# ParBLiSS/FastANI

Measured on NVIDIA H100. Metric: genome-pairs/sec (many-to-many, k=16, fragLen=3000), higher is better.
Workload: dtype u64

## Files before the change

fastani_b200/api.py:

```python
import ctypes as C
import os
import weakref
import numpy as np

_HERE = os.path.dirname(os.path.abspath(__file__))
_LIB_PATH = os.path.join(_HERE, "lib", "libfastani_b200.so")
_LIB = None

MAPPING_DTYPE = np.dtype([
    ("queryLen", "<i4"), ("refStartPos", "<i4"), ("refEndPos", "<i4"),
    ("queryStartPos", "<i4"), ("queryEndPos", "<i4"), ("refSeqId", "<i4"),
    ("querySeqId", "<i4"), ("nucIdentity", "<f4"), ("nucIdentityUpperBound", "<f4"),
    ("sketchSize", "<i4"), ("conservedSketches", "<i4")])
MINIMIZER_DTYPE = np.dtype([("hash", "<u4"), ("seqId", "<i4"), ("wpos", "<i4")])
CGI_DTYPE = np.dtype([("refGenomeId", "<i4"), ("qryGenomeId", "<i4"), ("countSeq", "<i4"),
                      ("totalQueryFragments", "<i4"), ("identity", "<f4")])
FRAG_DTYPE = np.dtype([("qryGenomeId", "<i4"), ("querySeqId", "<i4"), ("refSeqId", "<i4"), ("refStartPos", "<i4"),
                       ("identity", "<f4")])


class BaniError(RuntimeError):
    def __init__(self, code, msg):
        super().__init__("fastani_b200 error %d: %s" % (code, msg))
        self.code = code
# ... 45 lines not shown
        "bani_ctx_profile_read": (C.c_int, [vp, vp, vp, vp, vp, i32, P(i32)]),
        "bani_ctx_path_counts": (C.c_int, [vp, vp, vp, i32, P(i32)]),
        "bani_host_alloc": (C.c_int, [C.c_size_t, P(vp)]),
        "bani_host_free": (None, [vp]),
        "bani_genome_create": (C.c_int, [vp, i32, vp, vp, P(vp)]),
        "bani_genome_create_batch": (C.c_int, [vp, i32, vp, vp, vp, P(vp)]),
        "bani_pack_contig": (C.c_int, [vp, i64, vp, vp, vp, u64, P(u64)]),
        "bani_genome_create_packed_batch": (C.c_int, [vp, i32, vp, vp, vp, vp, vp, vp, vp, i32, P(vp)]),
        "bani_genome_destroy": (None, [vp]),
        "bani_genome_info": (C.c_int, [vp, P(i32), P(u64), P(u64), P(u64)]),
        "bani_genome_decode": (C.c_int, [vp, vp, i32, vp, i64]),
        "bani_index_build": (C.c_int, [vp, P(vp), i32, P(vp)]),
        "bani_index_destroy": (None, [vp]),
        "bani_index_stats": (C.c_int, [vp, P(u64), P(u64), P(u64), P(u64), P(u64)]),
        "bani_index_minimizers": (C.c_int, [vp, vp, vp, u64]),
        "bani_index_save": (C.c_int, [vp, vp, C.c_char_p]),
        "bani_index_load": (C.c_int, [vp, C.c_char_p, P(vp)]),
        "bani_index_contigs": (C.c_int, [vp, vp, u64, vp, u64]),
        "bani_qsketch_from_index": (C.c_int, [vp, vp, vp, i32, vp, P(vp)]),
        "bani_index_lookup": (C.c_int, [vp, vp, u32, vp, vp, u64, P(u64)]),
        "bani_map_genome": (C.c_int, [vp, vp, vp, P(vp), P(u64), P(u64), P(MapCounters)]),
        "bani_map_cgi": (C.c_int, [vp, vp, P(vp), i32, P(vp), P(u64), vp, P(MapCounters)]),
        "bani_device_count": (C.c_int, [P(i32)]),
        "bani_qsketch_create": (C.c_int, [vp, P(vp), i32, vp, vp, P(vp)]),
        "bani_qsketch_destroy": (None, [vp]),
        "bani_qsketch_info": (C.c_int, [vp, P(i32), P(u64), P(u64), P(u64)]),
        "bani_qsketch_export": (C.c_int, [vp, vp, vp, u64]),
        "bani_qsketch_import": (C.c_int, [vp, vp, u64, P(vp)]),
        "bani_qsketch_merge": (C.c_int, [vp, P(vp), i32, P(vp)]),
        "bani_map_cgi_sketch": (C.c_int, [vp, vp, P(vp), i32, P(vp), P(u64), P(MapCounters)]),
# ... 17 lines not shown
        "bani_qsketch_from_index_file": (C.c_int, [vp, C.c_char_p, vp, i32, vp, P(vp)]),
    }
    for name, (res, args) in sig.items():
        fn = getattr(L, name)
        fn.restype = res
        fn.argtypes = args
    _LIB = L
    return L


EXPORTED_SYMBOLS = [
    "bani_last_error", "bani_version", "bani_params_default", "bani_recommended_window_size", "bani_device_count",
    "bani_stat_min_hits_relaxed", "bani_stat_identity", "bani_ctx_create", "bani_ctx_destroy", "bani_ctx_params",
    "bani_ctx_sync", "bani_ctx_stream", "bani_ctx_launch_count", "bani_ctx_set_flag", "bani_ctx_profile_enable", "bani_ctx_profile_read", "bani_ctx_path_counts", "bani_host_alloc", "bani_host_free", "bani_genome_create",
    "bani_genome_create_batch", "bani_pack_contig", "bani_genome_create_packed_batch", "bani_genome_destroy", "bani_genome_info", "bani_genome_decode", "bani_index_build",
    "bani_index_destroy", "bani_index_stats", "bani_index_minimizers", "bani_index_save", "bani_index_load", "bani_index_contigs",
    "bani_qsketch_from_index", "bani_index_lookup", "bani_map_genome",
    "bani_map_cgi", "bani_free", "bani_synth_genome", "bani_qsketch_create", "bani_qsketch_destroy", "bani_qsketch_info",
    "bani_qsketch_export", "bani_qsketch_import", "bani_qsketch_merge", "bani_map_cgi_sketch", "bani_map_cgi_sketch_frags",
    "bani_index_build_budget", "bani_ctx_mem_stats", "bani_ctx_trim", "bani_ctx_plan_run", "bani_plan_run", "bani_run_working_set", "bani_index_footprint",
    "bani_map_working_set", "bani_index_budget", "bani_plan_chunks", "bani_qsketch_bytes_estimate", "bani_parse_byte_count",
    "bani_index_file_info", "bani_index_load_budget", "bani_qsketch_from_index_file"]


def _check(rc):
    if rc != 0:
        raise BaniError(rc, load_library().bani_last_error().decode())


def _records_from(ptr, n, dtype):
    out = np.empty(int(n), dtype)
# ... 293 lines not shown
        nc = st["n_contigs"]
        sk.metadata = [((names[c] if names else ""), int(cl[c])) for c in range(nc)]
        sk.sequencesByFileInfo = [int(x) for x in sbf[:st["n_genomes"]]]
        return sk

    def stats(self):
        a = [C.c_uint64() for _ in range(5)]
        _check(self.ctx.lib.bani_index_stats(self.h, *[C.byref(x) for x in a]))
        return dict(zip(("n_minimizers", "n_unique", "total_len", "n_contigs", "n_genomes"), [x.value for x in a]))

    def minimizerIndex(self):
        n = self.stats()["n_minimizers"]
        out = np.empty(max(n, 1), MINIMIZER_DTYPE)
        _check(self.ctx.lib.bani_index_minimizers(self.ctx.h, self.h, out.ctypes.data, n))
        return out[:n]

    def lookup(self, hash_value, cap=1 << 16):
        s = np.empty(cap, np.int32); w = np.empty(cap, np.int32); n = C.c_uint64()
        _check(self.ctx.lib.bani_index_lookup(self.ctx.h, self.h, int(hash_value), s.ctypes.data, w.ctypes.data, cap, C.byref(n)))
        m = min(n.value, cap)
        return list(zip(s[:m].tolist(), w[:m].tolist())), n.value

    def sanityCheck(self, maxRatioDiff):
        st = self.stats()
        if st["n_minimizers"] == 0 or st["n_unique"] == 0:
            return True, np.float32(0)
        hashRatio = np.float32(st["total_len"]) / np.float32(st["n_minimizers"])
        uniqHashRatio = np.float32(st["total_len"]) / np.float32(st["n_unique"])
        diff = np.float32(abs(hashRatio - uniqHashRatio))
        return (not diff > np.float32(maxRatioDiff)), diff
# ... 301 lines not shown
```

fastani_b200/csrc/budget.cpp:

```cpp
#include "common.cuh"
#include <algorithm>

namespace bani {

IndexFootprint index_footprint(uint64_t M, uint64_t Ub, uint64_t nC, uint64_t bits, uint64_t stagingCap)
{
  auto R = [](uint64_t b) { return (uint64_t)dev_round_size((size_t)b); };
  Ub = std::min(Ub, M);
  const uint64_t tables = R(4 * (nC + 1)) + R(4 * std::max<uint64_t>(nC, 1)) + R(4 * (nC + 1)) + (nC ? R(8 * nC) : 0);
  const uint64_t bitmap = R(4 * (bits / 32 + 1));
  const uint64_t desc = R(sizeof(SeqDesc) * std::max<uint64_t>(nC, 1));
  const uint64_t rec4 = R(4 * M);
  const uint64_t sketchTemp = R(4 * (nC + 1)) + R(2 * stagingCap + 8 * nC + 16);
  const uint64_t sketchStage = 2 * tables + 2 * bitmap + desc + 3 * R(4 * stagingCap) + sketchTemp + 3 * rec4;
  const uint64_t cubSort = R(8 * M + M / 4 + ((uint64_t)64 << 20));
  const uint64_t cubScan = R(M / 64 + ((uint64_t)1 << 20));
  const int fb = index_filt_bits(Ub);
  const uint64_t lookup = R(4 * Ub) + R(4 * (Ub + 1)) + R(4 * ((1ull << index_dir_bits(Ub)) + 1)) + R(32ull << index_tab_bits(Ub)) +
                          (fb ? R(4ull << (fb - 5)) : 0);
  const uint64_t l2 = R(16 * M) + R(8 * M) + R(8 * M) + R(4 * ((M + 1023) / 1024));
  const uint64_t base = tables + bitmap + 3 * rec4 + 2 * rec4;
  const uint64_t finishStage = base + 4 * rec4 + R(8) + std::max(std::max(cubSort, cubScan), lookup + l2);
  IndexFootprint f;
  f.peak = std::max(sketchStage, finishStage);
  f.resident = base + lookup + l2;
  return f;
}

uint64_t map_working_set(uint64_t deviceBytes, long long maxHitsPerPiece, long long eventBytesPerPiece)
{
  const uint64_t hits = 12ull * (uint64_t)std::max(1ll, maxHitsPerPiece);
  const uint64_t events = eventBytesPerPiece > 0 ? (uint64_t)eventBytesPerPiece : deviceBytes / 4;
  return hits + events + (3ull << 30);
}

uint64_t map_working_set_run(uint64_t deviceBytes, long long maxHitsPerPiece, long long eventBytesPerPiece, uint64_t queryHashes,
                             uint64_t queryFragments, uint64_t nQueries, uint64_t refBases, uint64_t nRefs, int w, int fragLen)
// ... 131 lines not shown
```

fastani_b200/csrc/capi.cu:

```cuda
#include "common.cuh"
#include <algorithm>
#include <cstring>
#include <cstdlib>

struct bani_ctx    { bani::Ctx c; };
struct bani_genome { bani::Genome g; };
struct bani_index  { bani::Index *ix; };
struct bani_qsketch { bani::QSketch *qs; };

namespace bani {
static thread_local std::string g_err;
void set_last_error(const std::string &m) { g_err = m; }
const char *const PATH_NAMES[NPATH] = {
  "l1.class0", "l1.class1", "l1.class2", "l1.class3", "l1.class4", "l1.class5", "l1.class6", "l1.class7", "l1.class8",
  "l1.class9", "l1.class10", "l1.class11", "l1.class12", "l1.device_wide",
  "lookup.walk_saturated", "lookup.walk_full_bucket",
  "l2.events_nt64", "l2.events_nt128", "l2.events_nt256", "l2.dir1024", "l2.dir4096", "l2.staged", "l2.direct",
  "l2.exact_at_bounds", "l2.exact_total",
  "piece.mapped", "piece.split_hits", "piece.split_events", "cgi.passes", "cgi.sparse"};
}

using namespace bani;

#define BANI_TRY try {
// ... 625 lines not shown
  const Index *ix = ixh->ix;
  if (cap < ix->M) fail(BANI_ERR_ARG, "output buffer too small (%llu < %llu)", (unsigned long long)cap, (unsigned long long)ix->M);
  BANI_CUDA(cudaSetDevice(ctx->c.device));
  const size_t M = ix->M;
  if (!M) return BANI_OK;
  std::vector<uint32_t> h(M); std::vector<int32_t> s(M), w(M);
  BANI_CUDA(cudaStreamSynchronize(ctx->c.stream));
  BANI_CUDA(cudaMemcpy(h.data(), ix->hash.p, 4 * M, cudaMemcpyDeviceToHost));
  BANI_CUDA(cudaMemcpy(s.data(), ix->seqId.p, 4 * M, cudaMemcpyDeviceToHost));
  BANI_CUDA(cudaMemcpy(w.data(), ix->wpos.p, 4 * M, cudaMemcpyDeviceToHost));
  for (size_t i = 0; i < M; i++) { out[i].hash = h[i]; out[i].seqId = s[i]; out[i].wpos = w[i]; }
  return BANI_OK;
  BANI_CATCH
}

int bani_index_lookup(bani_ctx *ctx, const bani_index *ixh, uint32_t hash, int32_t *seqId, int32_t *wpos, uint64_t cap, uint64_t *n)
{
  BANI_TRY
  if (!ctx || !ixh || !ixh->ix || !n) fail(BANI_ERR_ARG, "null argument");
  const Index *ix = ixh->ix;
  BANI_CUDA(cudaSetDevice(ctx->c.device));
  BANI_CUDA(cudaStreamSynchronize(ctx->c.stream));
  *n = 0;
  if (!ix->U) return BANI_OK;
  const uint32_t b = hash >> (32 - ix->dirBits);
  uint32_t d[2];
  BANI_CUDA(cudaMemcpy(d, ix->dir.p + b, 8, cudaMemcpyDeviceToHost));
  if (d[1] <= d[0]) return BANI_OK;
  std::vector<uint32_t> keys(d[1] - d[0]);
  BANI_CUDA(cudaMemcpy(keys.data(), ix->ukeys.p + d[0], 4 * keys.size(), cudaMemcpyDeviceToHost));
// ... 210 lines not shown
```

fastani_b200/csrc/common.cuh:

```cuda
#pragma once
#include <cuda_runtime.h>
#include <stdint.h>
#include <string>
#include <vector>
#include <memory>
#include <map>
#include <stdexcept>
#include <cstdio>
#include <cstdarg>
#include <chrono>
#include "../../include/fastani_b200.h"

namespace bani {

struct Error : std::runtime_error {
  int code;
  Error(int c, const std::string &m) : std::runtime_error(m), code(c) {}
};

void set_last_error(const std::string &m);

[[noreturn]] inline void fail(int code, const char *fmt, ...)
{
  char buf[512];
// ... 340 lines not shown
                  int64_t len, uint8_t *hostOut);

size_t cub_sort_pairs_u32_temp(size_t n);
void   cub_sort_pairs_u32(void *temp, size_t tempBytes, const uint32_t *kin, uint32_t *kout,
                          const uint32_t *vin, uint32_t *vout, size_t n, int endBit, cudaStream_t s);
size_t cub_sort_keys_u64_temp(size_t n);
void   cub_sort_keys_u64(void *temp, size_t tempBytes, const uint64_t *kin, uint64_t *kout, size_t n,
                         int beginBit, int endBit, cudaStream_t s);
size_t cub_sort_pairs_u64_u32_temp(size_t n);
void   cub_sort_pairs_u64_u32(void *temp, size_t tempBytes, const uint64_t *kin, uint64_t *kout,
                              const uint32_t *vin, uint32_t *vout, size_t n, int endBit, cudaStream_t s);
size_t cub_scan_u32_temp(size_t n);
void   cub_exclusive_sum_u32(void *temp, size_t tempBytes, const uint32_t *in, uint32_t *out, size_t n, cudaStream_t s);
size_t cub_scan_u64_temp(size_t n);
void   cub_exclusive_sum_u32_to_u64(void *temp, size_t tempBytes, const uint32_t *in, uint64_t *out, size_t n, cudaStream_t s);

}
```

fastani_b200/csrc/cubops.cu:

```cuda
#include <cub/cub.cuh>
#include "common.cuh"

namespace bani {

size_t cub_sort_pairs_u32_temp(size_t n)
{
  size_t b = 0;
  cub::DeviceRadixSort::SortPairs(nullptr, b, (const uint32_t *)nullptr, (uint32_t *)nullptr,
                                  (const uint32_t *)nullptr, (uint32_t *)nullptr, n);
  return b;
}
void cub_sort_pairs_u32(void *temp, size_t tempBytes, const uint32_t *kin, uint32_t *kout,
                        const uint32_t *vin, uint32_t *vout, size_t n, int endBit, cudaStream_t s)
{
  BANI_CUDA(cub::DeviceRadixSort::SortPairs(temp, tempBytes, kin, kout, vin, vout, n, 0, endBit, s));
}
size_t cub_sort_keys_u64_temp(size_t n)
{
  size_t b = 0;
  cub::DeviceRadixSort::SortKeys(nullptr, b, (const uint64_t *)nullptr, (uint64_t *)nullptr, n);
  return b;
}
void cub_sort_keys_u64(void *temp, size_t tempBytes, const uint64_t *kin, uint64_t *kout, size_t n,
                       int beginBit, int endBit, cudaStream_t s)
// ... 24 lines not shown
}
struct U32toU64 { __host__ __device__ uint64_t operator()(uint32_t x) const { return (uint64_t)x; } };
size_t cub_scan_u64_temp(size_t n)
{
  size_t b = 0;
  cub::TransformInputIterator<uint64_t, U32toU64, const uint32_t *> it((const uint32_t *)nullptr, U32toU64());
  cub::DeviceScan::ExclusiveSum(nullptr, b, it, (uint64_t *)nullptr, n);
  return b;
}
void cub_exclusive_sum_u32_to_u64(void *temp, size_t tempBytes, const uint32_t *in, uint64_t *out, size_t n, cudaStream_t s)
{
  cub::TransformInputIterator<uint64_t, U32toU64, const uint32_t *> it(in, U32toU64());
  BANI_CUDA(cub::DeviceScan::ExclusiveSum(temp, tempBytes, it, out, n, s));
}

}
```

fastani_b200/csrc/index.cu:

```cuda
#include "common.cuh"
#include <algorithm>

namespace bani {

static inline unsigned nblk(uint64_t n, int t = 256) { return (unsigned)((n + t - 1) / t); }

__global__ void iota_kernel(uint32_t *v, uint64_t n)
{
  uint64_t i = (uint64_t)blockIdx.x * blockDim.x + threadIdx.x;
  if (i < n) v[i] = (uint32_t)i;
}

__global__ void head_flags_kernel(const uint32_t *sh, uint64_t n, uint32_t *head)
{
  uint64_t i = (uint64_t)blockIdx.x * blockDim.x + threadIdx.x;
  if (i < n) head[i] = (i == 0 || sh[i] != sh[i - 1]) ? 1u : 0u;
}

__global__ void unique_scatter_kernel(const uint32_t *sh, const uint32_t *head, const uint32_t *scan, uint64_t n,
                                      uint32_t *ukeys, uint32_t *uoff, unsigned long long *o_U)
{
  uint64_t i = (uint64_t)blockIdx.x * blockDim.x + threadIdx.x;
  if (i >= n) return;
  if (head[i]) { ukeys[scan[i]] = sh[i]; uoff[scan[i]] = (uint32_t)i; }
  if (i == n - 1) { uint32_t U = scan[i] + head[i]; *o_U = U; }
}

__global__ void links_kernel(const uint32_t *sh, const uint32_t *posIdx, uint64_t n, uint32_t *link)
{
  uint64_t i = (uint64_t)blockIdx.x * blockDim.x + threadIdx.x;
  if (i >= n) return;
  const uint32_t h = sh[i];
  const bool hasPrev = i > 0 && sh[i - 1] == h, hasNext = i + 1 < n && sh[i + 1] == h;
  if (!hasPrev && !hasNext) return;
  const uint32_t r = posIdx[i];
  uint32_t pd = 0xFFFFu, nd = 0xFFFFu;
  if (hasPrev) pd = min(r - posIdx[i - 1], 0xFFFFu);
  if (hasNext) nd = min(posIdx[i + 1] - r, 0xFFFFu);
  if (pd != 0xFFFFu || nd != 0xFFFFu) link[r] = (pd << 16) | nd;
}

__global__ void zip_records_kernel(const uint32_t *hash, const int32_t *wpos, const uint32_t *link, const int32_t *seqId,
                                   const uint32_t *contigRecOff, int cmw, uint64_t n, uint4 *rec, int2 *pos8, uint2 *rec8)
{
  uint64_t i64 = (uint64_t)blockIdx.x * blockDim.x + threadIdx.x;
  if (i64 >= n) return;
  const uint32_t i = (uint32_t)i64;
  const int32_t wx = wpos[i];
  const int seq = seqId[i];
  const uint32_t lo = contigRecOff[seq], hi = contigRecOff[seq + 1];
  uint32_t back = 0, fwd = 0xFFFFu, tie = 0;
  if (cmw >= 2) {
    {
      const int32_t v = wx - cmw + 1;
      uint32_t l = (i - lo > (uint32_t)cmw) ? i - (uint32_t)cmw : lo, h = i;
      while (l < h) { uint32_t m = (l + h) >> 1; if (wpos[m] <= v) l = m + 1; else h = m; }
      back = min(i - l + 1, 0xFFFFu);
    }
    if (i + 1 < hi) {
      const int32_t v = wpos[i + 1] + cmw - 1;
      uint32_t l = i + 1, h = (hi - i - 1 > (uint32_t)cmw + 1) ? i + 1 + (uint32_t)cmw + 1 : hi;
      while (l < h) { uint32_t m = (l + h) >> 1; if (wpos[m] < v) l = m + 1; else h = m; }
      fwd = min(l - i, 0xFFFEu);
      tie = (l < hi && wpos[l] == v) ? 1u : 0u;
    }
  }
  rec[i] = make_uint4(hash[i], (uint32_t)wx | (tie << 31), link[i], back | (fwd << 16));
  pos8[i] = make_int2(wx, seq);
  const uint32_t pd = link[i] >> 16, nd = link[i] & 0xFFFFu;
  const uint32_t f14 = fwd == 0xFFFFu ? 0x3FFFu : min(fwd, 0x3FFEu);
  rec8[i] = make_uint2(hash[i], (back & 0x3FFFu) | (f14 << 14) | (tie << 28) | ((pd > back ? 1u : 0u) << 29) | ((nd >= fwd ? 1u : 0u) << 30));
}

__global__ void block_link_max_kernel(const uint4 *rec, uint64_t n, uint32_t *blkMax)
{
  __shared__ uint32_t s_b, s_f;
  if (threadIdx.x == 0) { s_b = 0; s_f = 0; }
  __syncthreads();
  uint32_t mb = 0, mf = 0;
  for (int j = 0; j < 4; j++) {
    const uint64_t i = (uint64_t)blockIdx.x * 1024 + (uint64_t)j * 256 + threadIdx.x;
    if (i < n) {
      const uint32_t w = rec[i].w, back = w & 0xFFFFu, fwd = w >> 16;
      if (back >= 0x3FFFu || (fwd != 0xFFFFu && fwd >= 0x3FFFu)) { mb = 0xFFFFu; mf = 0xFFFFu; }
      else { mb = max(mb, back); if (fwd != 0xFFFFu) mf = max(mf, fwd); }
    }
  }
  atomicMax(&s_b, mb); atomicMax(&s_f, mf);
  __syncthreads();
  if (threadIdx.x == 0) blkMax[blockIdx.x] = min(s_b, 0xFFFFu) | (min(s_f, 0xFFFFu) << 16);
}

__global__ void dir_fill_kernel(const uint32_t *ukeys, uint32_t U, int dirBits, uint32_t *dir)
{
  uint32_t b = blockIdx.x * blockDim.x + threadIdx.x;
  if (b > (1u << dirBits)) return;
  uint32_t lo = 0, hi = U;
  if (b == (1u << dirBits)) lo = U;
  else { const uint32_t v = b << (32 - dirBits); while (lo < hi) { uint32_t mid = (lo + hi) >> 1; if (ukeys[mid] < v) lo = mid + 1; else hi = mid; } }
  dir[b] = lo;
}

__global__ void table_fill_kernel(const uint32_t *ukeys, const uint32_t *uoff, uint32_t U, uint32_t mask, uint2 *tab,
                                  uint32_t *filt, uint32_t filtMask)
{
  const uint32_t u = blockIdx.x * blockDim.x + threadIdx.x;
  if (u >= U) return;
  const uint32_t h = ukeys[u], o = uoff[u], cnt = uoff[u + 1] - o;
  if (filt) atomicOr(&filt[(h & filtMask) >> 5], 1u << (h & 31u));
  const unsigned long long e = ((unsigned long long)o << 32) | (unsigned long long)((h & 0xFFFFFF00u) | min(cnt, 255u));
  unsigned long long *bp = reinterpret_cast<unsigned long long *>(tab + 4 * (size_t)(h & mask));
#pragma unroll
  for (int sl = 0; sl < 4; sl++) if (atomicCAS(bp + sl, 0ull, e) == 0ull) return;
}

__global__ void fill_u32(uint32_t *p, uint32_t v, uint64_t n)
{
  uint64_t i = (uint64_t)blockIdx.x * blockDim.x + threadIdx.x;
  if (i < n) p[i] = v;
}

static unsigned long long index_contig_tables(Ctx *ctx, Index *ix, const std::vector<int32_t> &contigGenome)
{
  cudaStream_t st = ctx->stream;
  const int fragLen = ix->fragLen;
  const int32_t nC = (int32_t)ix->contigLen.size();
  std::vector<uint32_t> binOff(1, 0);
  std::vector<unsigned long long> bitBase;
// ... 33 lines not shown
  BANI_CUDA(cudaMemsetAsync(ix->dir.p, 0, 4 * ((1u << ix->dirBits) + 1), st));
  ix->ukeys.alloc(1, st); ix->uoff.alloc(2, st); ix->posIdx.alloc(1, st);
  BANI_CUDA(cudaMemsetAsync(ix->uoff.p, 0, 8, st));
  ix->tabBits = 8; ix->tab.alloc((size_t)4 << ix->tabBits, st);
  BANI_CUDA(cudaMemsetAsync(ix->tab.p, 0, ix->tab.bytes(), st));
  ix->hash.alloc(1, st); ix->wpos.alloc(1, st); ix->seqId.alloc(1, st); ix->link.alloc(1, st);
  BANI_CUDA(cudaStreamSynchronize(st));
}

static void index_finish(Ctx *ctx, Index *ix)
{
  cudaStream_t st = ctx->stream;
  const uint64_t M = ix->M;
  ix->link.alloc(M, st);
  ix->posIdx.alloc(M, st);
  DevBuf<uint32_t> sortedHash(M, st), iota(M, st), head(M, st), scan(M, st);
  DevBuf<unsigned long long> d_U(1, st);
  {
    Stage sg(ctx, "index_sort", 24.0 * M);
    iota_kernel<<<nblk(M), 256, 0, st>>>(iota.p, M);
    ctx->launches++;
    size_t tb = cub_sort_pairs_u32_temp(M);
    DevBuf<uint8_t> tmp(tb, st);
    cub_sort_pairs_u32(tmp.p, tb, ix->hash.p, sortedHash.p, iota.p, ix->posIdx.p, M, 32, st);
  }
  Stage sgc(ctx, "index_compact", 16.0 * M);
  head_flags_kernel<<<nblk(M), 256, 0, st>>>(sortedHash.p, M, head.p);
  ctx->launches++;
  {
    size_t tb = cub_scan_u32_temp(M);
    DevBuf<uint8_t> tmp(tb, st);
    cub_exclusive_sum_u32(tmp.p, tb, head.p, scan.p, M, st);
  }
  uint32_t lastScan = 0, lastHead = 0;
  BANI_CUDA(cudaMemcpyAsync(&lastScan, scan.p + (M - 1), 4, cudaMemcpyDeviceToHost, st));
  BANI_CUDA(cudaMemcpyAsync(&lastHead, head.p + (M - 1), 4, cudaMemcpyDeviceToHost, st));
  BANI_CUDA(cudaStreamSynchronize(st));
  const uint64_t U = (uint64_t)lastScan + lastHead;
  ix->U = U;
  ix->ukeys.alloc(U, st); ix->uoff.alloc(U + 1, st);
  unique_scatter_kernel<<<nblk(M), 256, 0, st>>>(sortedHash.p, head.p, scan.p, M, ix->ukeys.p, ix->uoff.p, d_U.p);
  ctx->launches++;
  { uint32_t Mu = (uint32_t)M; BANI_CUDA(cudaMemcpyAsync(ix->uoff.p + U, &Mu, 4, cudaMemcpyHostToDevice, st)); }
  BANI_CUDA(cudaMemsetAsync(ix->link.p, 0xFF, 4 * (size_t)M, st));
  links_kernel<<<nblk(M), 256, 0, st>>>(sortedHash.p, ix->posIdx.p, M, ix->link.p);
  ctx->launches++;
  const int bits = index_dir_bits(U);
  ix->dirBits = bits;
  ix->dir.alloc((1u << bits) + 1, st);
  dir_fill_kernel<<<nblk((1ull << bits) + 1), 256, 0, st>>>(ix->ukeys.p, (uint32_t)U, bits, ix->dir.p);
  ctx->launches++;
  {
    const int tb = index_tab_bits(U);
    ix->tabBits = tb;
    ix->tab.alloc((size_t)4 << tb, st);
    BANI_CUDA(cudaMemsetAsync(ix->tab.p, 0, ix->tab.bytes(), st));
    const int fb = index_filt_bits(U);
    ix->filtBits = fb;
    if (fb) { ix->filt.alloc((size_t)1 << (fb - 5), st); BANI_CUDA(cudaMemsetAsync(ix->filt.p, 0, ix->filt.bytes(), st)); }
    table_fill_kernel<<<nblk(U), 256, 0, st>>>(ix->ukeys.p, ix->uoff.p, (uint32_t)U, (1u << tb) - 1u, ix->tab.p,
                                               ix->filt.p, fb ? (uint32_t)((1ull << fb) - 1ull) : 0u);
    ctx->launches++;
  }
  ix->rec.alloc(M, st);
  ix->cmw = ix->fragLen - (ix->w - 1) - (ix->k - 1);
  ix->pos8.alloc(M, st); ix->rec8.alloc(M, st);
  zip_records_kernel<<<nblk(M), 256, 0, st>>>(ix->hash.p, ix->wpos.p, ix->link.p, ix->seqId.p, ix->contigRecOff.p, ix->cmw, M, ix->rec.p, ix->pos8.p, ix->rec8.p);
  ctx->launches++;
  ix->blkMax.alloc((size_t)((M + 1023) / 1024), st);
  block_link_max_kernel<<<(unsigned)((M + 1023) / 1024), 256, 0, st>>>(ix->rec.p, M, ix->blkMax.p);
  ctx->launches++;
  sgc.stop();
  BANI_CUDA(cudaGetLastError());
  BANI_CUDA(cudaStreamSynchronize(st));
}

struct GenomeSpan { uint64_t nC = 0, pos = 0, bits = 0; };
static GenomeSpan genome_span(const Genome *G, int k)
{
  GenomeSpan s;
  s.nC = (uint64_t)G->nContigs;
  for (int c = 0; c < G->nContigs; c++) {
    if (G->len[c] >= k) s.pos += (uint64_t)(G->len[c] - k + 1);
    s.bits += ((uint64_t)G->len[c] + 31) & ~31ull;
  }
// ... 98 lines not shown
  const int32_t nC = (int32_t)desc.size();
  ctx->mark("index_build: enter + contig loop");
  const unsigned long long totalBits = index_contig_tables(ctx, ix.get(), contigGenome);
  ctx->mark("index_build: contig tables");

  if (nC == 0 || totalPos == 0) { index_make_empty(ctx, ix.get()); return ix.release(); }

  ix->validBits.alloc((size_t)(totalBits / 32) + 1, st);
  BANI_CUDA(cudaMemsetAsync(ix->validBits.p, 0, ix->validBits.bytes(), st));
  DevBuf<SeqDesc> d_desc(nC, st);
  BANI_CUDA(cudaMemcpyAsync(d_desc.p, desc.data(), sizeof(SeqDesc) * (size_t)nC, cudaMemcpyHostToDevice, st));

  uint64_t cap = index_staging_cap(totalPos, w);
  uint64_t M = 0;
  {
    DevBuf<uint32_t> th; DevBuf<int32_t> tw, ts;
    std::vector<std::pair<int32_t, int32_t>> groups;
    std::vector<const Genome *> groupHead;
    {
      int32_t c = 0;
      for (int g = 0; g < nRefs; g++) {
        const Genome *G = refs[g];
        const bool newGroup = groups.empty() || G->blk != groupHead.back()->blk;
        if (newGroup) { groups.push_back({c, c}); groupHead.push_back(G); }
        c += G->nContigs; groups.back().second = c;
      }
    }
    for (int attempt = 0; attempt < 2; attempt++) {
      if (cap > 0xfffffff0ull) fail(BANI_ERR_LIMIT, "more than 2^32 minimizers in one index shard");
      th.alloc(cap, st); tw.alloc(cap, st); ts.alloc(cap, st);
      Stage sg(ctx, "ref_sketch", (double)ix->totalLen / 4.0);
      M = 0;
      for (size_t gi = 0; gi < groups.size(); gi++) {
        const int32_t ca = groups[gi].first, cb = groups[gi].second;
        groupHead[gi]->wait_ready(st);
        M += sketch_sequences(ctx, d_desc.p + ca, cb - ca, ix->contigLen.data() + ca, 0, th.p, tw.p, ts.p, cap, ix->contigRecOff.p + ca,
                              ix->validBits.p, ix->contigBitBase.p + ca, M);
        if (M > 0xfffffff0ull) fail(BANI_ERR_LIMIT, "more than 2^32 minimizers in one index shard");
      }
      sg.bytes((double)ix->totalLen / 4.0 + 12.0 * (double)M);
      ctx->mark("index_build: sketched");
      if (M <= cap) break;
      if (budget) {
        uint32_t r1 = 0;
        BANI_CUDA(cudaMemcpyAsync(&r1, ix->contigRecOff.p + ix->seqsByFile[0], 4, cudaMemcpyDeviceToHost, st));
        BANI_CUDA(cudaStreamSynchronize(st));
        if (r1 <= cap) break;
        if (index_footprint(r1, r1, (uint64_t)nC, totalBits, r1).peak > maxBytes)
          fail(BANI_ERR_LIMIT, "reference genome 0 of this chunk (%llu minimizers) does not fit the index budget of %llu bytes",
               (unsigned long long)r1, (unsigned long long)maxBytes);
        cap = r1;
        continue;
      }
      cap = M;
    }
    d_desc.release();
    if (budget) M = index_cut(ctx, ix.get(), refs, contigGenome, span, std::min(M, cap), cap, maxBytes, nTaken);
    if (M > 0xfffffff0ull) fail(BANI_ERR_LIMIT, "more than 2^32 minimizers in one index shard");
    ix->M = M;
    if (M == 0) { index_make_empty(ctx, ix.get()); return ix.release(); }
    ix->hash.alloc(M, st); ix->wpos.alloc(M, st); ix->seqId.alloc(M, st);
    BANI_CUDA(cudaMemcpyAsync(ix->hash.p, th.p, 4 * M, cudaMemcpyDeviceToDevice, st));
    BANI_CUDA(cudaMemcpyAsync(ix->wpos.p, tw.p, 4 * M, cudaMemcpyDeviceToDevice, st));
    BANI_CUDA(cudaMemcpyAsync(ix->seqId.p, ts.p, 4 * M, cudaMemcpyDeviceToDevice, st));
  }
  index_finish(ctx, ix.get());
  ctx->mark("index_build: finished");
  return ix.release();
}

Index *index_build(Ctx *ctx, Genome *const *refs, int32_t nRefs)
{
  int32_t n = 0;
  return index_build_impl(ctx, refs, nRefs, 0, &n);
}

template <typename F>
static Index *with_peak(Ctx *ctx, uint64_t *peakBytes, F &&make)
{
// ... 7 lines not shown
  dev_mem_peak_set(ctx->device, std::max(peak0, peak));
  *peakBytes = peak > live0 ? peak - live0 : 0;
  return ix;
}

Index *index_build_budget(Ctx *ctx, Genome *const *refs, int32_t nRefs, uint64_t maxBytes, int32_t *nTaken, uint64_t *peakBytes)
{
  if (nRefs < 1) fail(BANI_ERR_ARG, "a budgeted index build needs at least one genome");
  if (maxBytes == 0) fail(BANI_ERR_ARG, "the index budget must be positive");
  return with_peak(ctx, peakBytes, [&] { return index_build_impl(ctx, refs, nRefs, maxBytes, nTaken); });
}


static constexpr uint64_t IX_MAGIC = 0x32584449494e4142ull;
static constexpr uint64_t IX_HEADER_BYTES = 128;

__global__ void seqid_fill_kernel(const uint32_t *contigRecOff, int32_t nC, int32_t *seqId)
{
  const int c = blockIdx.x;
  if (c >= nC) return;
  const uint32_t a = contigRecOff[c], b = contigRecOff[c + 1];
  for (uint32_t i = a + threadIdx.x; i < b; i += blockDim.x) seqId[i] = c;
}

static uint64_t word_sum(const void *p, size_t bytes)
{
  const uint32_t *w = (const uint32_t *)p;
  uint64_t s = 0;
  for (size_t i = 0; i < bytes / 4; i++) s += w[i];
  return s;
}

namespace {
struct File {
  FILE *f = nullptr; std::string path; uint64_t sum = 0;
  File(const char *p, const char *mode) : f(fopen(p, mode)), path(p) { if (!f) fail(BANI_ERR_ARG, "cannot open %s", p); }
  ~File() { if (f) fclose(f); }
  void write(const void *p, size_t n) { if (n && fwrite(p, 1, n, f) != n) fail(BANI_ERR_INTERNAL, "write error on %s", path.c_str()); sum += word_sum(p, n); }
// ... 322 lines not shown
```

fastani_b200/csrc/sketch.cu:

```cuda
#include "common.cuh"

namespace bani {

static constexpr int SK_THREADS = 256;
static constexpr int SK_P = 16;
static constexpr int SK_SLOTS = SK_THREADS * SK_P;
static constexpr int SK_WMAX = 1024;
static constexpr int SK_KMAX = 32;
static constexpr int SK_ASCII = SK_SLOTS + SK_KMAX + 64;
#define KIDX(q) ((q) + ((q) >> 4))
static constexpr int SK_KEYS = SK_SLOTS + SK_SLOTS / 16;

struct SketchArgs {
  const SeqDesc *desc; const uint32_t *tileOff;
  int32_t nSeq; uint32_t nTiles;
  int32_t uniformTiles;
  int k, w, tileLen;
  uint32_t *o_hash; int32_t *o_wpos; int32_t *o_seqId; uint64_t cap;
  uint32_t *o_segStart;
  unsigned long long *tileState;
  unsigned long long *o_total;
  uint32_t *o_validBits; const unsigned long long *bitBase;
  unsigned long long recBase;
};
// ... 99 lines not shown
  }
}

__device__ __forceinline__ uint64_t min64(uint64_t a, uint64_t b) { return a < b ? a : b; }

__device__ __forceinline__ void expand8(uint32_t x, uint32_t &b0, uint32_t &b1)
{
  x = (x | (x << 8)) & 0x00FF00FFu;
  x = (x | (x << 4)) & 0x0F0F0F0Fu;
  x = (x | (x << 2)) & 0x33333333u;
  b0 = __byte_perm(0x54474341u, 0u, x & 0xFFFFu);
  b1 = __byte_perm(0x54474341u, 0u, x >> 16);
}

template <int KT, int G>
__global__ void __launch_bounds__(SK_THREADS)
sketch_kernel(const SketchArgs a)
{
  __shared__ __align__(16) uint8_t  s_ascii[SK_ASCII];
  __shared__ __align__(16) uint64_t s_key[SK_KEYS];
  __shared__ uint16_t s_vmask[SK_THREADS];
  __shared__ uint32_t s_wsum[SK_THREADS / 32];
  __shared__ unsigned long long s_base;

  const int tid = threadIdx.x, lane = tid & 31, wid = tid >> 5;
  const uint32_t tile = blockIdx.x;
  const int k = KT > 0 ? KT : a.k, w = a.w;

  int seq, t0;
  if (a.uniformTiles > 0) { seq = (int)(tile / (uint32_t)a.uniformTiles); t0 = (int)(tile % (uint32_t)a.uniformTiles) * a.tileLen; }
  else {
// ... 242 lines not shown
```

include/fastani_b200.h:

```cpp
#ifndef FASTANI_B200_H
#define FASTANI_B200_H

#include <stdint.h>
#include <stddef.h>

#ifdef __cplusplus
extern "C" {
#endif

#define BANI_API __attribute__((visibility("default")))

typedef enum {
  BANI_OK = 0,
  BANI_ERR_ARG = -1,
  BANI_ERR_CUDA = -2,
  BANI_ERR_NOMEM = -3,
  BANI_ERR_LIMIT = -4,
  BANI_ERR_INTERNAL = -5
} bani_status;

typedef struct {
  int32_t  kmer_size;
  int32_t  window_size;
  int32_t  frag_len;
// ... 99 lines not shown
                               uint64_t budget, int32_t *chunk_end, int32_t *n_chunks);
BANI_API int  bani_qsketch_bytes_estimate(uint64_t len, int32_t w, int32_t frag_len, uint64_t *bytes);
BANI_API int  bani_plan_run(uint64_t free_bytes, uint64_t device_bytes, int64_t max_hits_per_piece, int64_t event_bytes_per_piece,
                            uint64_t index_budget, uint64_t query_budget, int32_t k, int32_t w, int32_t frag_len,
                            const uint64_t *ref_len, const int32_t *ref_contigs, int32_t n_refs, const uint64_t *query_len,
                            const uint64_t *query_sketch_bytes, int32_t n_queries, int32_t *chunk_end, int32_t *n_chunks,
                            int32_t *block_end, int32_t *n_blocks, uint64_t *index_budget_used);
BANI_API int  bani_ctx_plan_run(bani_ctx *ctx, uint64_t index_budget, uint64_t query_budget, const uint64_t *ref_len, const int32_t *ref_contigs, int32_t n_refs,
                                const uint64_t *query_len, const uint64_t *query_sketch_bytes, int32_t n_queries,
                                int32_t *chunk_end, int32_t *n_chunks, int32_t *block_end, int32_t *n_blocks,
                                uint64_t *index_budget_used);
BANI_API int  bani_parse_byte_count(const char *s, uint64_t *out);
BANI_API int  bani_index_stats(const bani_index *ix, uint64_t *n_minimizers, uint64_t *n_unique,
                               uint64_t *total_len, uint64_t *n_contigs, uint64_t *n_genomes);
BANI_API int  bani_index_minimizers(bani_ctx *ctx, const bani_index *ix, bani_minimizer *out, uint64_t cap);
BANI_API int  bani_index_lookup(bani_ctx *ctx, const bani_index *ix, uint32_t hash,
                                int32_t *seqId, int32_t *wpos, uint64_t cap, uint64_t *n);

BANI_API int  bani_index_save(bani_ctx *ctx, const bani_index *ix, const char *path);
BANI_API int  bani_index_load(bani_ctx *ctx, const char *path, bani_index **out);
BANI_API int  bani_index_contigs(const bani_index *ix, int32_t *contig_len, uint64_t cap_contigs, int32_t *seqs_by_file, uint64_t cap_genomes);

BANI_API int  bani_index_file_info(const char *path, int32_t *version, int32_t *k, int32_t *w, int32_t *frag_len, int32_t *n_genomes,
                                   uint64_t *n_contigs, uint64_t *n_minimizers, int32_t *genome_contigs, uint64_t *genome_len,
                                   uint64_t *genome_records, uint64_t *genome_bits, uint64_t cap_genomes, int32_t *contig_len,
                                   uint64_t cap_contigs);
BANI_API int  bani_index_load_budget(bani_ctx *ctx, const char *path, int32_t first_genome, uint64_t max_bytes, bani_index **out,
                                     int32_t *n_taken, uint64_t *peak_bytes);

BANI_API int  bani_map_genome(bani_ctx *ctx, const bani_index *ix, const bani_genome *query,
// ... 36 lines not shown
```

Baseline: 2.112 million.

## Streamline index build: CUB unique, fused zip/blkMax, seqId fill, sketch bounds

Replaces the head-flag, scan and scatter sequence in index compaction with a CUB run-count followed by UniqueByKey. Fuses the block link-max reduction into the record zip kernel, which now handles 1024 elements per block with warp reductions. Drops the per-minimizer seqId staging buffer from sketching and rebuilds seqId from contig offsets. It also adds min-blocks 4 to the sketch kernel's launch bounds, which may cause register spills, and adds an index-array export API. These mostly cut index-build launches, memory and traffic, which is a small share of many-to-many mapping throughput.

New measurement: 2.150 million, median of 6. 1.02x the previous value.

```diff
diff --git a/fastani_b200/api.py b/fastani_b200/api.py
--- a/fastani_b200/api.py
+++ b/fastani_b200/api.py
@@ -83,6 +83,7 @@
         "bani_index_destroy": (None, [vp]),
         "bani_index_stats": (C.c_int, [vp, P(u64), P(u64), P(u64), P(u64), P(u64)]),
         "bani_index_minimizers": (C.c_int, [vp, vp, vp, u64]),
+        "bani_index_array": (C.c_int, [vp, vp, C.c_char_p, vp, u64, P(u64)]),
         "bani_index_save": (C.c_int, [vp, vp, C.c_char_p]),
         "bani_index_load": (C.c_int, [vp, C.c_char_p, P(vp)]),
         "bani_index_contigs": (C.c_int, [vp, vp, u64, vp, u64]),
@@ -130,7 +131,7 @@
     "bani_stat_min_hits_relaxed", "bani_stat_identity", "bani_ctx_create", "bani_ctx_destroy", "bani_ctx_params",
     "bani_ctx_sync", "bani_ctx_stream", "bani_ctx_launch_count", "bani_ctx_set_flag", "bani_ctx_profile_enable", "bani_ctx_profile_read", "bani_ctx_path_counts", "bani_host_alloc", "bani_host_free", "bani_genome_create",
     "bani_genome_create_batch", "bani_pack_contig", "bani_genome_create_packed_batch", "bani_genome_destroy", "bani_genome_info", "bani_genome_decode", "bani_index_build",
-    "bani_index_destroy", "bani_index_stats", "bani_index_minimizers", "bani_index_save", "bani_index_load", "bani_index_contigs",
+    "bani_index_destroy", "bani_index_stats", "bani_index_minimizers", "bani_index_array", "bani_index_save", "bani_index_load", "bani_index_contigs",
     "bani_qsketch_from_index", "bani_index_lookup", "bani_map_genome",
     "bani_map_cgi", "bani_free", "bani_synth_genome", "bani_qsketch_create", "bani_qsketch_destroy", "bani_qsketch_info",
     "bani_qsketch_export", "bani_qsketch_import", "bani_qsketch_merge", "bani_map_cgi_sketch", "bani_map_cgi_sketch_frags",
@@ -454,6 +455,13 @@
         out = np.empty(max(n, 1), MINIMIZER_DTYPE)
         _check(self.ctx.lib.bani_index_minimizers(self.ctx.h, self.h, out.ctypes.data, n))
         return out[:n]
+
+    def array(self, name, dtype):
+        n = C.c_uint64()
+        _check(self.ctx.lib.bani_index_array(self.ctx.h, self.h, name.encode(), None, 0, C.byref(n)))
+        out = np.empty(max(n.value, 1), np.uint8)
+        _check(self.ctx.lib.bani_index_array(self.ctx.h, self.h, name.encode(), out.ctypes.data, n.value, C.byref(n)))
+        return out[:n.value].view(dtype)
 
     def lookup(self, hash_value, cap=1 << 16):
         s = np.empty(cap, np.int32); w = np.empty(cap, np.int32); n = C.c_uint64()
diff --git a/fastani_b200/csrc/budget.cpp b/fastani_b200/csrc/budget.cpp
--- a/fastani_b200/csrc/budget.cpp
+++ b/fastani_b200/csrc/budget.cpp
@@ -12,15 +12,16 @@
   const uint64_t desc = R(sizeof(SeqDesc) * std::max<uint64_t>(nC, 1));
   const uint64_t rec4 = R(4 * M);
   const uint64_t sketchTemp = R(4 * (nC + 1)) + R(2 * stagingCap + 8 * nC + 16);
-  const uint64_t sketchStage = 2 * tables + 2 * bitmap + desc + 3 * R(4 * stagingCap) + sketchTemp + 3 * rec4;
+  const uint64_t sketchStage = 2 * tables + 2 * bitmap + desc + 2 * R(4 * stagingCap) + sketchTemp + 3 * rec4;
   const uint64_t cubSort = R(8 * M + M / 4 + ((uint64_t)64 << 20));
-  const uint64_t cubScan = R(M / 64 + ((uint64_t)1 << 20));
+  const uint64_t cubUnique = R(M / 64 + ((uint64_t)1 << 20));
   const int fb = index_filt_bits(Ub);
   const uint64_t lookup = R(4 * Ub) + R(4 * (Ub + 1)) + R(4 * ((1ull << index_dir_bits(Ub)) + 1)) + R(32ull << index_tab_bits(Ub)) +
                           (fb ? R(4ull << (fb - 5)) : 0);
   const uint64_t l2 = R(16 * M) + R(8 * M) + R(8 * M) + R(4 * ((M + 1023) / 1024));
   const uint64_t base = tables + bitmap + 3 * rec4 + 2 * rec4;
-  const uint64_t finishStage = base + 4 * rec4 + R(8) + std::max(std::max(cubSort, cubScan), lookup + l2);
+  const uint64_t compact = cubUnique + R(4) + R(4 * Ub) + R(4 * (Ub + 1));
+  const uint64_t finishStage = base + rec4 + std::max(std::max(rec4 + cubSort, compact), lookup + l2);
   IndexFootprint f;
   f.peak = std::max(sketchStage, finishStage);
   f.resident = base + lookup + l2;
diff --git a/fastani_b200/csrc/capi.cu b/fastani_b200/csrc/capi.cu
--- a/fastani_b200/csrc/capi.cu
+++ b/fastani_b200/csrc/capi.cu
@@ -663,6 +663,29 @@
   BANI_CATCH
 }
 
+int bani_index_array(bani_ctx *ctx, const bani_index *ixh, const char *name, void *out, uint64_t cap_bytes, uint64_t *n_bytes)
+{
+  BANI_TRY
+  if (!ctx || !ixh || !ixh->ix || !name || !n_bytes) fail(BANI_ERR_ARG, "null argument");
+  const Index *ix = ixh->ix;
+  const std::string nm(name);
+  const void *p = nullptr; size_t b = 0; bool found = false;
+  auto pick = [&](const char *n, const auto &buf) { if (nm == n) { p = buf.p; b = buf.bytes(); found = true; } };
+  pick("hash", ix->hash); pick("wpos", ix->wpos); pick("seqId", ix->seqId); pick("link", ix->link); pick("posIdx", ix->posIdx);
+  pick("ukeys", ix->ukeys); pick("uoff", ix->uoff); pick("dir", ix->dir); pick("rec", ix->rec); pick("pos8", ix->pos8);
+  pick("rec8", ix->rec8); pick("blkMax", ix->blkMax); pick("contigRecOff", ix->contigRecOff); pick("tab", ix->tab);
+  pick("filt", ix->filt); pick("validBits", ix->validBits);
+  if (!found) fail(BANI_ERR_ARG, "unknown index array '%s'", name);
+  *n_bytes = b;
+  if (!out) return BANI_OK;
+  if (cap_bytes < b) fail(BANI_ERR_ARG, "output buffer too small (%llu < %llu)", (unsigned long long)cap_bytes, (unsigned long long)b);
+  BANI_CUDA(cudaSetDevice(ctx->c.device));
+  BANI_CUDA(cudaStreamSynchronize(ctx->c.stream));
+  if (b) BANI_CUDA(cudaMemcpy(out, p, b, cudaMemcpyDeviceToHost));
+  return BANI_OK;
+  BANI_CATCH
+}
+
 int bani_index_lookup(bani_ctx *ctx, const bani_index *ixh, uint32_t hash, int32_t *seqId, int32_t *wpos, uint64_t cap, uint64_t *n)
 {
   BANI_TRY
diff --git a/fastani_b200/csrc/common.cuh b/fastani_b200/csrc/common.cuh
--- a/fastani_b200/csrc/common.cuh
+++ b/fastani_b200/csrc/common.cuh
@@ -378,5 +378,10 @@
 void   cub_exclusive_sum_u32(void *temp, size_t tempBytes, const uint32_t *in, uint32_t *out, size_t n, cudaStream_t s);
 size_t cub_scan_u64_temp(size_t n);
 void   cub_exclusive_sum_u32_to_u64(void *temp, size_t tempBytes, const uint32_t *in, uint64_t *out, size_t n, cudaStream_t s);
-
-}
+size_t cub_count_runs_u32_temp(size_t n);
+void   cub_count_runs_u32(void *temp, size_t tempBytes, const uint32_t *keys, uint32_t *o_runs, size_t n, cudaStream_t s);
+size_t cub_unique_u32_temp(size_t n);
+void   cub_unique_u32(void *temp, size_t tempBytes, const uint32_t *keys, uint32_t *o_keys, uint32_t *o_first, uint32_t *o_count,
+                      size_t n, cudaStream_t s);
+
+}
diff --git a/fastani_b200/csrc/cubops.cu b/fastani_b200/csrc/cubops.cu
--- a/fastani_b200/csrc/cubops.cu
+++ b/fastani_b200/csrc/cubops.cu
@@ -62,4 +62,34 @@
   BANI_CUDA(cub::DeviceScan::ExclusiveSum(temp, tempBytes, it, out, n, s));
 }
 
+struct RunHead {
+  const uint32_t *k;
+  __host__ __device__ uint32_t operator()(uint32_t i) const { return (i == 0 || k[i] != k[i - 1]) ? 1u : 0u; }
+};
+size_t cub_count_runs_u32_temp(size_t n)
+{
+  size_t b = 0;
+  cub::TransformInputIterator<uint32_t, RunHead, cub::CountingInputIterator<uint32_t>> it(cub::CountingInputIterator<uint32_t>(0), RunHead{nullptr});
+  cub::DeviceReduce::Sum(nullptr, b, it, (uint32_t *)nullptr, (uint32_t)n);
+  return b;
 }
+void cub_count_runs_u32(void *temp, size_t tempBytes, const uint32_t *keys, uint32_t *o_runs, size_t n, cudaStream_t s)
+{
+  cub::TransformInputIterator<uint32_t, RunHead, cub::CountingInputIterator<uint32_t>> it(cub::CountingInputIterator<uint32_t>(0), RunHead{keys});
+  BANI_CUDA(cub::DeviceReduce::Sum(temp, tempBytes, it, o_runs, (uint32_t)n, s));
+}
+size_t cub_unique_u32_temp(size_t n)
+{
+  size_t b = 0;
+  cub::DeviceSelect::UniqueByKey(nullptr, b, (const uint32_t *)nullptr, cub::CountingInputIterator<uint32_t>(0), (uint32_t *)nullptr,
+                                 (uint32_t *)nullptr, (uint32_t *)nullptr, (uint32_t)n);
+  return b;
+}
+void cub_unique_u32(void *temp, size_t tempBytes, const uint32_t *keys, uint32_t *o_keys, uint32_t *o_first, uint32_t *o_count,
+                    size_t n, cudaStream_t s)
+{
+  BANI_CUDA(cub::DeviceSelect::UniqueByKey(temp, tempBytes, keys, cub::CountingInputIterator<uint32_t>(0), o_keys, o_first, o_count,
+                                           (uint32_t)n, s));
+}
+
+}
diff --git a/fastani_b200/csrc/index.cu b/fastani_b200/csrc/index.cu
--- a/fastani_b200/csrc/index.cu
+++ b/fastani_b200/csrc/index.cu
@@ -9,21 +9,6 @@
 {
   uint64_t i = (uint64_t)blockIdx.x * blockDim.x + threadIdx.x;
   if (i < n) v[i] = (uint32_t)i;
-}
-
-__global__ void head_flags_kernel(const uint32_t *sh, uint64_t n, uint32_t *head)
-{
-  uint64_t i = (uint64_t)blockIdx.x * blockDim.x + threadIdx.x;
-  if (i < n) head[i] = (i == 0 || sh[i] != sh[i - 1]) ? 1u : 0u;
-}
-
-__global__ void unique_scatter_kernel(const uint32_t *sh, const uint32_t *head, const uint32_t *scan, uint64_t n,
-                                      uint32_t *ukeys, uint32_t *uoff, unsigned long long *o_U)
-{
-  uint64_t i = (uint64_t)blockIdx.x * blockDim.x + threadIdx.x;
-  if (i >= n) return;
-  if (head[i]) { ukeys[scan[i]] = sh[i]; uoff[scan[i]] = (uint32_t)i; }
-  if (i == n - 1) { uint32_t U = scan[i] + head[i]; *o_U = U; }
 }
 
 __global__ void links_kernel(const uint32_t *sh, const uint32_t *posIdx, uint64_t n, uint32_t *link)
@@ -40,55 +25,54 @@
   if (pd != 0xFFFFu || nd != 0xFFFFu) link[r] = (pd << 16) | nd;
 }
 
-__global__ void zip_records_kernel(const uint32_t *hash, const int32_t *wpos, const uint32_t *link, const int32_t *seqId,
-                                   const uint32_t *contigRecOff, int cmw, uint64_t n, uint4 *rec, int2 *pos8, uint2 *rec8)
-{
-  uint64_t i64 = (uint64_t)blockIdx.x * blockDim.x + threadIdx.x;
-  if (i64 >= n) return;
-  const uint32_t i = (uint32_t)i64;
-  const int32_t wx = wpos[i];
-  const int seq = seqId[i];
-  const uint32_t lo = contigRecOff[seq], hi = contigRecOff[seq + 1];
-  uint32_t back = 0, fwd = 0xFFFFu, tie = 0;
-  if (cmw >= 2) {
-    {
-      const int32_t v = wx - cmw + 1;
-      uint32_t l = (i - lo > (uint32_t)cmw) ? i - (uint32_t)cmw : lo, h = i;
-      while (l < h) { uint32_t m = (l + h) >> 1; if (wpos[m] <= v) l = m + 1; else h = m; }
-      back = min(i - l + 1, 0xFFFFu);
-    }
-    if (i + 1 < hi) {
-      const int32_t v = wpos[i + 1] + cmw - 1;
-      uint32_t l = i + 1, h = (hi - i - 1 > (uint32_t)cmw + 1) ? i + 1 + (uint32_t)cmw + 1 : hi;
-      while (l < h) { uint32_t m = (l + h) >> 1; if (wpos[m] < v) l = m + 1; else h = m; }
-      fwd = min(l - i, 0xFFFEu);
-      tie = (l < hi && wpos[l] == v) ? 1u : 0u;
-    }
-  }
-  rec[i] = make_uint4(hash[i], (uint32_t)wx | (tie << 31), link[i], back | (fwd << 16));
-  pos8[i] = make_int2(wx, seq);
-  const uint32_t pd = link[i] >> 16, nd = link[i] & 0xFFFFu;
-  const uint32_t f14 = fwd == 0xFFFFu ? 0x3FFFu : min(fwd, 0x3FFEu);
-  rec8[i] = make_uint2(hash[i], (back & 0x3FFFu) | (f14 << 14) | (tie << 28) | ((pd > back ? 1u : 0u) << 29) | ((nd >= fwd ? 1u : 0u) << 30));
-}
-
-__global__ void block_link_max_kernel(const uint4 *rec, uint64_t n, uint32_t *blkMax)
-{
-  __shared__ uint32_t s_b, s_f;
-  if (threadIdx.x == 0) { s_b = 0; s_f = 0; }
+__global__ void __launch_bounds__(256) zip_records_kernel(const uint32_t *hash, const int32_t *wpos, const uint32_t *link,
+                                                          const int32_t *seqId, const uint32_t *contigRecOff, int cmw, uint64_t n,
+                                                          uint4 *rec, int2 *pos8, uint2 *rec8, uint32_t *blkMax)
+{
+  __shared__ uint32_t s_b[8], s_f[8];
+  uint32_t mb = 0, mf = 0;
+#pragma unroll 1
+  for (int jj = 0; jj < 4; jj++) {
+    const uint64_t i64 = (uint64_t)blockIdx.x * 1024 + (uint64_t)jj * 256 + threadIdx.x;
+    if (i64 >= n) break;
+    const uint32_t i = (uint32_t)i64;
+    const int32_t wx = wpos[i];
+    const int seq = seqId[i];
+    const uint32_t lo = contigRecOff[seq], hi = contigRecOff[seq + 1];
+    uint32_t back = 0, fwd = 0xFFFFu, tie = 0;
+    if (cmw >= 2) {
+      {
+        const int32_t v = wx - cmw + 1;
+        uint32_t l = (i - lo > (uint32_t)cmw) ? i - (uint32_t)cmw : lo, h = i;
+        while (l < h) { uint32_t m = (l + h) >> 1; if (wpos[m] <= v) l = m + 1; else h = m; }
+        back = min(i - l + 1, 0xFFFFu);
+      }
+      if (i + 1 < hi) {
+        const int32_t v = wpos[i + 1] + cmw - 1;
+        uint32_t l = i + 1, h = (hi - i - 1 > (uint32_t)cmw + 1) ? i + 1 + (uint32_t)cmw + 1 : hi;
+        while (l < h) { uint32_t m = (l + h) >> 1; if (wpos[m] < v) l = m + 1; else h = m; }
+        fwd = min(l - i, 0xFFFEu);
+        tie = (l < hi && wpos[l] == v) ? 1u : 0u;
+      }
+    }
+    const uint32_t hx = hash[i], lk = link[i];
+    rec[i] = make_uint4(hx, (uint32_t)wx | (tie << 31), lk, back | (fwd << 16));
+    pos8[i] = make_int2(wx, seq);
+    const uint32_t pd = lk >> 16, nd = lk & 0xFFFFu;
+    const uint32_t f14 = fwd == 0xFFFFu ? 0x3FFFu : min(fwd, 0x3FFEu);
+    rec8[i] = make_uint2(hx, (back & 0x3FFFu) | (f14 << 14) | (tie << 28) | ((pd > back ? 1u : 0u) << 29) | ((nd >= fwd ? 1u : 0u) << 30));
+    if (back >= 0x3FFFu || (fwd != 0xFFFFu && fwd >= 0x3FFFu)) { mb = 0xFFFFu; mf = 0xFFFFu; }
+    else { mb = max(mb, back); if (fwd != 0xFFFFu) mf = max(mf, fwd); }
+  }
+  mb = __reduce_max_sync(0xffffffffu, mb); mf = __reduce_max_sync(0xffffffffu, mf);
+  if ((threadIdx.x & 31) == 0) { s_b[threadIdx.x >> 5] = mb; s_f[threadIdx.x >> 5] = mf; }
   __syncthreads();
-  uint32_t mb = 0, mf = 0;
-  for (int j = 0; j < 4; j++) {
-    const uint64_t i = (uint64_t)blockIdx.x * 1024 + (uint64_t)j * 256 + threadIdx.x;
-    if (i < n) {
-      const uint32_t w = rec[i].w, back = w & 0xFFFFu, fwd = w >> 16;
-      if (back >= 0x3FFFu || (fwd != 0xFFFFu && fwd >= 0x3FFFu)) { mb = 0xFFFFu; mf = 0xFFFFu; }
-      else { mb = max(mb, back); if (fwd != 0xFFFFu) mf = max(mf, fwd); }
-    }
-  }
-  atomicMax(&s_b, mb); atomicMax(&s_f, mf);
-  __syncthreads();
-  if (threadIdx.x == 0) blkMax[blockIdx.x] = min(s_b, 0xFFFFu) | (min(s_f, 0xFFFFu) << 16);
+  if (threadIdx.x == 0) {
+    uint32_t b = 0, f = 0;
+#pragma unroll
+    for (int q = 0; q < 8; q++) { b = max(b, s_b[q]); f = max(f, s_f[q]); }
+    blkMax[blockIdx.x] = min(b, 0xFFFFu) | (min(f, 0xFFFFu) << 16);
+  }
 }
 
 __global__ void dir_fill_kernel(const uint32_t *ukeys, uint32_t U, int dirBits, uint32_t *dir)
@@ -112,6 +96,14 @@
   unsigned long long *bp = reinterpret_cast<unsigned long long *>(tab + 4 * (size_t)(h & mask));
 #pragma unroll
   for (int sl = 0; sl < 4; sl++) if (atomicCAS(bp + sl, 0ull, e) == 0ull) return;
+}
+
+__global__ void seqid_fill_kernel(const uint32_t *contigRecOff, int32_t nC, int32_t *seqId)
+{
+  const int c = blockIdx.x;
+  if (c >= nC) return;
+  const uint32_t a = contigRecOff[c], b = contigRecOff[c + 1];
+  for (uint32_t i = a + threadIdx.x; i < b; i += blockDim.x) seqId[i] = c;
 }
 
 __global__ void fill_u32(uint32_t *p, uint32_t v, uint64_t n)
@@ -175,9 +167,9 @@
   const uint64_t M = ix->M;
   ix->link.alloc(M, st);
   ix->posIdx.alloc(M, st);
-  DevBuf<uint32_t> sortedHash(M, st), iota(M, st), head(M, st), scan(M, st);
-  DevBuf<unsigned long long> d_U(1, st);
-  {
+  DevBuf<uint32_t> sortedHash(M, st);
+  {
+    DevBuf<uint32_t> iota(M, st);
     Stage sg(ctx, "index_sort", 24.0 * M);
     iota_kernel<<<nblk(M), 256, 0, st>>>(iota.p, M);
     ctx->launches++;
@@ -186,22 +178,19 @@
     cub_sort_pairs_u32(tmp.p, tb, ix->hash.p, sortedHash.p, iota.p, ix->posIdx.p, M, 32, st);
   }
   Stage sgc(ctx, "index_compact", 16.0 * M);
-  head_flags_kernel<<<nblk(M), 256, 0, st>>>(sortedHash.p, M, head.p);
-  ctx->launches++;
-  {
-    size_t tb = cub_scan_u32_temp(M);
+  uint32_t U32 = 0;
+  {
+    DevBuf<uint32_t> d_U(1, st);
+    const size_t tb = std::max(cub_count_runs_u32_temp(M), cub_unique_u32_temp(M));
     DevBuf<uint8_t> tmp(tb, st);
-    cub_exclusive_sum_u32(tmp.p, tb, head.p, scan.p, M, st);
-  }
-  uint32_t lastScan = 0, lastHead = 0;
-  BANI_CUDA(cudaMemcpyAsync(&lastScan, scan.p + (M - 1), 4, cudaMemcpyDeviceToHost, st));
-  BANI_CUDA(cudaMemcpyAsync(&lastHead, head.p + (M - 1), 4, cudaMemcpyDeviceToHost, st));
-  BANI_CUDA(cudaStreamSynchronize(st));
-  const uint64_t U = (uint64_t)lastScan + lastHead;
+    cub_count_runs_u32(tmp.p, tb, sortedHash.p, d_U.p, M, st);
+    BANI_CUDA(cudaMemcpyAsync(&U32, d_U.p, 4, cudaMemcpyDeviceToHost, st));
+    BANI_CUDA(cudaStreamSynchronize(st));
+    ix->ukeys.alloc(U32, st); ix->uoff.alloc((size_t)U32 + 1, st);
+    cub_unique_u32(tmp.p, tb, sortedHash.p, ix->ukeys.p, ix->uoff.p, d_U.p, M, st);
+  }
+  const uint64_t U = U32;
   ix->U = U;
-  ix->ukeys.alloc(U, st); ix->uoff.alloc(U + 1, st);
-  unique_scatter_kernel<<<nblk(M), 256, 0, st>>>(sortedHash.p, head.p, scan.p, M, ix->ukeys.p, ix->uoff.p, d_U.p);
-  ctx->launches++;
   { uint32_t Mu = (uint32_t)M; BANI_CUDA(cudaMemcpyAsync(ix->uoff.p + U, &Mu, 4, cudaMemcpyHostToDevice, st)); }
   BANI_CUDA(cudaMemsetAsync(ix->link.p, 0xFF, 4 * (size_t)M, st));
   links_kernel<<<nblk(M), 256, 0, st>>>(sortedHash.p, ix->posIdx.p, M, ix->link.p);
@@ -226,10 +215,9 @@
   ix->rec.alloc(M, st);
   ix->cmw = ix->fragLen - (ix->w - 1) - (ix->k - 1);
   ix->pos8.alloc(M, st); ix->rec8.alloc(M, st);
-  zip_records_kernel<<<nblk(M), 256, 0, st>>>(ix->hash.p, ix->wpos.p, ix->link.p, ix->seqId.p, ix->contigRecOff.p, ix->cmw, M, ix->rec.p, ix->pos8.p, ix->rec8.p);
-  ctx->launches++;
   ix->blkMax.alloc((size_t)((M + 1023) / 1024), st);
-  block_link_max_kernel<<<(unsigned)((M + 1023) / 1024), 256, 0, st>>>(ix->rec.p, M, ix->blkMax.p);
+  zip_records_kernel<<<(unsigned)((M + 1023) / 1024), 256, 0, st>>>(ix->hash.p, ix->wpos.p, ix->link.p, ix->seqId.p, ix->contigRecOff.p,
+                                                                    ix->cmw, M, ix->rec.p, ix->pos8.p, ix->rec8.p, ix->blkMax.p);
   ctx->launches++;
   sgc.stop();
   BANI_CUDA(cudaGetLastError());
@@ -358,7 +346,7 @@
   uint64_t cap = index_staging_cap(totalPos, w);
   uint64_t M = 0;
   {
-    DevBuf<uint32_t> th; DevBuf<int32_t> tw, ts;
+    DevBuf<uint32_t> th; DevBuf<int32_t> tw;
     std::vector<std::pair<int32_t, int32_t>> groups;
     std::vector<const Genome *> groupHead;
     {
@@ -372,13 +360,13 @@
     }
     for (int attempt = 0; attempt < 2; attempt++) {
       if (cap > 0xfffffff0ull) fail(BANI_ERR_LIMIT, "more than 2^32 minimizers in one index shard");
-      th.alloc(cap, st); tw.alloc(cap, st); ts.alloc(cap, st);
+      th.alloc(cap, st); tw.alloc(cap, st);
       Stage sg(ctx, "ref_sketch", (double)ix->totalLen / 4.0);
       M = 0;
       for (size_t gi = 0; gi < groups.size(); gi++) {
         const int32_t ca = groups[gi].first, cb = groups[gi].second;
         groupHead[gi]->wait_ready(st);
-        M += sketch_sequences(ctx, d_desc.p + ca, cb - ca, ix->contigLen.data() + ca, 0, th.p, tw.p, ts.p, cap, ix->contigRecOff.p + ca,
+        M += sketch_sequences(ctx, d_desc.p + ca, cb - ca, ix->contigLen.data() + ca, 0, th.p, tw.p, nullptr, cap, ix->contigRecOff.p + ca,
                               ix->validBits.p, ix->contigBitBase.p + ca, M);
         if (M > 0xfffffff0ull) fail(BANI_ERR_LIMIT, "more than 2^32 minimizers in one index shard");
       }
@@ -406,7 +394,8 @@
     ix->hash.alloc(M, st); ix->wpos.alloc(M, st); ix->seqId.alloc(M, st);
     BANI_CUDA(cudaMemcpyAsync(ix->hash.p, th.p, 4 * M, cudaMemcpyDeviceToDevice, st));
     BANI_CUDA(cudaMemcpyAsync(ix->wpos.p, tw.p, 4 * M, cudaMemcpyDeviceToDevice, st));
-    BANI_CUDA(cudaMemcpyAsync(ix->seqId.p, ts.p, 4 * M, cudaMemcpyDeviceToDevice, st));
+    seqid_fill_kernel<<<(unsigned)ix->nContigs, 512, 0, st>>>(ix->contigRecOff.p, ix->nContigs, ix->seqId.p);
+    ctx->launches++;
   }
   index_finish(ctx, ix.get());
   ctx->mark("index_build: finished");
@@ -444,14 +433,6 @@
 
 static constexpr uint64_t IX_MAGIC = 0x32584449494e4142ull;
 static constexpr uint64_t IX_HEADER_BYTES = 128;
-
-__global__ void seqid_fill_kernel(const uint32_t *contigRecOff, int32_t nC, int32_t *seqId)
-{
-  const int c = blockIdx.x;
-  if (c >= nC) return;
-  const uint32_t a = contigRecOff[c], b = contigRecOff[c + 1];
-  for (uint32_t i = a + threadIdx.x; i < b; i += blockDim.x) seqId[i] = c;
-}
 
 static uint64_t word_sum(const void *p, size_t bytes)
 {
diff --git a/fastani_b200/csrc/sketch.cu b/fastani_b200/csrc/sketch.cu
--- a/fastani_b200/csrc/sketch.cu
+++ b/fastani_b200/csrc/sketch.cu
@@ -137,7 +137,7 @@
 }
 
 template <int KT, int G>
-__global__ void __launch_bounds__(SK_THREADS)
+__global__ void __launch_bounds__(SK_THREADS, 4)
 sketch_kernel(const SketchArgs a)
 {
   __shared__ __align__(16) uint8_t  s_ascii[SK_ASCII];
diff --git a/include/fastani_b200.h b/include/fastani_b200.h
--- a/include/fastani_b200.h
+++ b/include/fastani_b200.h
@@ -137,6 +137,7 @@
 BANI_API int  bani_index_stats(const bani_index *ix, uint64_t *n_minimizers, uint64_t *n_unique,
                                uint64_t *total_len, uint64_t *n_contigs, uint64_t *n_genomes);
 BANI_API int  bani_index_minimizers(bani_ctx *ctx, const bani_index *ix, bani_minimizer *out, uint64_t cap);
+BANI_API int  bani_index_array(bani_ctx *ctx, const bani_index *ix, const char *name, void *out, uint64_t cap_bytes, uint64_t *n_bytes);
 BANI_API int  bani_index_lookup(bani_ctx *ctx, const bani_index *ix, uint32_t hash,
                                 int32_t *seqId, int32_t *wpos, uint64_t cap, uint64_t *n);
 
```
